# benfred/implicit

Hardware: AMD Instinct MI355X
Metric: ALS user+item updates/sec per iteration (factors=128); top-k recs/sec (higher is better)
Workload: dtype f32; 1 GPU; BASELINE configs[2]: last.fm-360K-shaped synthetic CSR, ALS CG cg_steps=3; users=358868, items=292385, nnz=17308340, factors=128, solver=cg, cg_steps=3

## Files before the change

implicit_amd/csrc/als_cg_fixup.hip:

```cpp
#include <type_traits>

#include "als_qtile.h"
#include "common.h"

namespace imp {

template <int F, typename ST>
__global__ __launch_bounds__(256) void als_cg_fault_fixup_kernel(const unsigned *__restrict__ fault_count,
                                                                 const unsigned *__restrict__ fault_rows, int capacity,
                                                                 const int32_t *__restrict__ indptr,
                                                                 const int32_t *__restrict__ indices,
                                                                 const float *__restrict__ data, ST *__restrict__ X,
                                                                 const ST *__restrict__ Y, const float *__restrict__ A0, int cg_steps,
                                                                 unsigned long long *total) {
  constexpr int FC = F / 64, WAVES = 4, U = 4;
  __shared__ float vecs[WAVES][F];
  const int n = min((int)fault_count[0], capacity);
  if (n == 0) return;
  if (blockIdx.x == 0 && threadIdx.x == 0) __hip_atomic_fetch_add(total, (unsigned long long)n, __ATOMIC_RELAXED, __HIP_MEMORY_SCOPE_SYSTEM);
  const int lane = threadIdx.x & 63, wave = threadIdx.x >> 6;
  float *vec = vecs[wave];
  auto load_vec = [&](const ST *row, float (&v)[FC]) {
#pragma unroll
    for (int c = 0; c < FC; ++c) v[c] = load1(row + FC * lane + c);
  };
  auto apply = [&](bool first, int rb, int re, const float (&v)[FC], float (&acc)[FC]) {
#pragma unroll
    for (int c = 0; c < FC; ++c) vec[FC * lane + c] = v[c];
#pragma unroll
    for (int c = 0; c < FC; ++c) acc[c] = 0.f;
    for (int j = 0; j < F; ++j) {
      const float vj = vec[j];
#pragma unroll
      for (int c = 0; c < FC; ++c) acc[c] = fmaf(A0[(size_t)j * F + FC * lane + c], vj, acc[c]);
    }
    if (first) {
#pragma unroll
      for (int c = 0; c < FC; ++c) acc[c] = -acc[c];
    }
    for (int k0 = rb; k0 < re; k0 += U) {
      float conf[U], y[U][FC];
#pragma unroll
      for (int q = 0; q < U; ++q) {
        const int k = min(k0 + q, re - 1);
        conf[q] = data[k];
        load_vec(Y + (size_t)indices[k] * F, y[q]);
      }
#pragma unroll
      for (int q = 0; q < U; ++q) {
        if (k0 + q < re) {
          const float d = wave_allsum(dot_local<FC>(y[q], v));
          const float cm1 = fabsf(conf[q]) - 1.f;
          const float w = first ? fmaxf(conf[q], 0.f) - cm1 * d : cm1 * d;
#pragma unroll
          for (int c = 0; c < FC; ++c) acc[c] = fmaf(w, y[q][c], acc[c]);
        }
      }
    }
  };
  for (int i = blockIdx.x * WAVES + wave; i < n; i += gridDim.x * WAVES) {
    const int u = (int)fault_rows[i];
    const int rb = indptr[u], re = indptr[u + 1];
    ST *xrow = X + (size_t)u * F;
    float x[FC], r[FC], p[FC], Ap[FC];
    load_vec(xrow, x);
    apply(true, rb, re, x, r);
#pragma unroll
    for (int c = 0; c < FC; ++c) p[c] = r[c];
    float rsold = wave_allsum(dot_local<FC>(r, r));
    if (rsold < 1e-20f) continue;
    for (int it = 0; it < cg_steps; ++it) {
      apply(false, rb, re, p, Ap);
      const float alpha = rsold / wave_allsum(dot_local<FC>(p, Ap));
#pragma unroll
      for (int c = 0; c < FC; ++c) {
        x[c] = fmaf(alpha, p[c], x[c]);
        r[c] = fmaf(-alpha, Ap[c], r[c]);
      }
      const float rsnew = wave_allsum(dot_local<FC>(r, r));
      if (rsnew < 1e-20f) break;
      const float beta = rsnew / rsold;
#pragma unroll
      for (int c = 0; c < FC; ++c) p[c] = fmaf(beta, p[c], r[c]);
      rsold = rsnew;
    }
#pragma unroll
    for (int c = 0; c < FC; ++c) store1(xrow + FC * lane + c, x[c]);
  }
}

unsigned long long *fixup_total() {
  auto &c = ctx();
  if (!c.fixup_total) {
    IMP_CHECK_HIP(hipHostMalloc(reinterpret_cast<void **>(&c.fixup_total), sizeof(unsigned long long), hipHostMallocMapped));
    *c.fixup_total = 0ull;
  }
  return c.fixup_total;
}

template <int F, typename T>
void launch_cg_fixup(const unsigned *count, const unsigned *rows, int capacity, const imp_csr *C, T *X, const T *Y, const float *A0,
                     int cg_steps) {
  if (capacity <= 0) return;
  IMP_PROF("als_cg_fixup");
  als_cg_fault_fixup_kernel<F, T><<<std::min((capacity + 3) / 4, ctx().num_cus * 2), 256, 0, stream()>>>(
      count, rows, capacity, C->indptr.data(), C->indices.data(), C->data.data(), X, Y, A0, cg_steps, fixup_total());
  IMP_CHECK_HIP(hipGetLastError());
}
template void launch_cg_fixup<64, float>(const unsigned *, const unsigned *, int, const imp_csr *, float *, const float *, const float *, int);
template void launch_cg_fixup<128, float>(const unsigned *, const unsigned *, int, const imp_csr *, float *, const float *, const float *, int);
template void launch_cg_fixup<64, __half>(const unsigned *, const unsigned *, int, const imp_csr *, __half *, const __half *, const float *, int);
template void launch_cg_fixup<128, __half>(const unsigned *, const unsigned *, int, const imp_csr *, __half *, const __half *, const float *, int);


}
```

implicit_amd/csrc/als_cg_nm.hip:

```cpp
#include "als_qf_common.h"
#include "common.h"
#include "wave_ops.h"

namespace imp {

namespace {

typedef _Float16 half8 __attribute__((ext_vector_type(8)));
typedef _Float16 half2v __attribute__((ext_vector_type(2)));
typedef float f32x16 __attribute__((ext_vector_type(16)));
typedef float f32x4v __attribute__((ext_vector_type(4)));
typedef unsigned u32x4 __attribute__((ext_vector_type(4)));

template <int F> struct NmShape;
template <> struct NmShape<128> {
  static constexpr int M = 32, KG = 2, NACC = 16;
  using acc_t = f32x16;
  __device__ static __forceinline__ acc_t mfma(half8 a, half8 b, acc_t c) { return __builtin_amdgcn_mfma_f32_32x32x16_f16(a, b, c, 0, 0, 0); }
  __device__ static __forceinline__ int row(int lane, int e) { return (e & 3) + 8 * (e >> 2) + 4 * (lane >> 5); }
  __device__ static __forceinline__ int col(int lane) { return lane & 31; }
};
template <> struct NmShape<64> {
  static constexpr int M = 16, KG = 4, NACC = 4;
  using acc_t = f32x4v;
// ... 22 lines not shown

__device__ __forceinline__ void split_pair(float x0, float x1, unsigned &hi, unsigned &lo) {
  const f32x2 v = {x0, x1};
  const half2v h = __builtin_convertvector(v, half2v);
  const f32x2 r = v - __builtin_convertvector(h, f32x2);
  const half2v l = __builtin_convertvector(r, half2v);
  hi = __builtin_bit_cast(unsigned, h);
  lo = __builtin_bit_cast(unsigned, l);
}
__device__ __forceinline__ unsigned pack_pair(float x0, float x1) {
  const f32x2 v = {x0, x1};
  return __builtin_bit_cast(unsigned, __builtin_convertvector(v, half2v));
}
__device__ __forceinline__ float comp(const float4 &v, int c) { return c == 0 ? v.x : c == 1 ? v.y : c == 2 ? v.z : v.w; }

template <int F> __global__ void nm_gram_image_kernel(const float *__restrict__ A0, float *__restrict__ img, int *__restrict__ ctl,
                                                      float y_rows, int forced_k, float reg = 0.f) {
  using L = NmLayout<F>;
  if (blockIdx.x == 0 && threadIdx.x < 64) {
    float d = 0.f;
    for (int j = threadIdx.x; j < F; j += 64) d = fmaxf(d, A0[(size_t)j * F + j]);
    d = wave_allmax(d);
    if (threadIdx.x == 0) {
      int k = 0;
      const float rms = sqrtf((d + reg) / fmaxf(y_rows, 1.f));
      if (rms > 0.f && rms < 8.f) k = min((int)floorf(log2f(8.f / rms)), 16);
      ctl[0] = 0;
      ctl[1] = forced_k >= 0 ? forced_k : k;
      ctl[2] = 0;
      ctl[3] = 0;
    }
  }
  for (int e = blockIdx.x * blockDim.x + threadIdx.x; e < L::IMG; e += gridDim.x * blockDim.x) {
    const int n = e % L::TS, m = (e / L::TS) % L::M, t = e / (L::TS * L::M);
    img[e] = n < L::M ? A0[(size_t)(4 * m + t / 4) * F + 4 * n + t % 4] + ((m == n && t / 4 == t % 4) ? reg : 0.f) : 0.f;
  }
}

__device__ __forceinline__ void lds_barrier() { asm volatile("s_waitcnt lgkmcnt(0)\n\ts_barrier" ::: "memory"); }

template <int F, typename T, bool TRIM = false>
__device__ __forceinline__ void nm_build(const int32_t *__restrict__ indices, const float *__restrict__ data, const T *__restrict__ Y,
                                         const float *__restrict__ gram_img, bool whole, int begin, int end, float *smem, float *bvec,
                                         int tid, int ko, int scale_k) {
  using S = NmShape<F>;
  using L = NmLayout<F>;
  constexpr bool kHalf = !std::is_same<T, float>::value;
  const int lane = tid & 63, wave = __builtin_amdgcn_readfirstlane(tid >> 6);
  const int a = lane % S::M, g = lane / S::M;
  const int first = wave < 2 ? 3 * wave : 2 * wave + 2;
  const int n_slots = wave < 2 ? 3 : 2;
  int tI[L::kSlots], tJ[L::kSlots];
#pragma unroll
  for (int k = 0; k < L::kSlots; ++k) {
    const int t = min(first + k, L::kTiles - 1);
    tI[k] = t < 1 ? 0 : t < 3 ? 1 : t < 6 ? 2 : 3;
    tJ[k] = t - tI[k] * (tI[k] + 1) / 2;
  }
// ... 196 lines not shown
      float v = b4[c];
      if constexpr (S::KG == 4) v += __shfl_xor(v, 16, 64);
      v += __shfl_xor(v, 32, 64);
      if (g == 0) bstage[wave * F + c * L::M + a] = v;
    }
    float *img = smem;
    const int n = S::col(lane);
#pragma unroll
    for (int k = 0; k < L::kSlots; ++k) {
      if (k < n_slots) {
        const int I = tI[k], J = tJ[k];
        float gv[S::NACC];
#pragma unroll
        for (int e = 0; e < S::NACC; ++e) gv[e] = 0.f;
        if (whole) {
#pragma unroll
          for (int e = 0; e < S::NACC; ++e) gv[e] = gram_img[L::at(I, J, S::row(lane, e), n)];
        }
#pragma unroll
        for (int e = 0; e < S::NACC; ++e) {
          const int m = S::row(lane, e);
          const float v = fmaf(acc[k][e], unscale2, gv[e]);
          img[L::at(I, J, m, n)] = v;
          if (I != J) img[L::at(J, I, n, m)] = v;
        }
      }
    }
  }
  __syncthreads();
}

template <int F, typename T>
// ... 221 lines not shown
    const float x2 = fmaf(-q3.z, x3, z.z) * q2.z;
    const float x1 = fmaf(-q3.y, x3, fmaf(-q2.y, x2, z.y)) * q1.y;
    const float x0 = fmaf(-q3.x, x3, fmaf(-q2.x, x2, fmaf(-q1.x, x1, z.x))) * q0.x;
    if (tid < 4 * kb) {
      const float *col = img + (size_t)(4 * kb) * LDL + tid;
      bvec[tid] = fmaf(-col[3 * LDL], x3, fmaf(-col[2 * LDL], x2, fmaf(-col[LDL], x1, fmaf(-col[0], x0, bvec[tid]))));
    }
    if (tid == 0) *reinterpret_cast<float4 *>(xs + 4 * kb) = make_float4(x0, x1, x2, x3);
    __syncthreads();
  }
  CHOL_TICK(4);
  if (tid < F) xrow[tid] = xs[tid];
  return false;
}

template <int F, typename T, bool CHOL = false>
__global__ __launch_bounds__(256, 2) void als_cg_nm_kernel(const LongPlanDev plan, const int32_t *__restrict__ indices,
                                                           const float *__restrict__ data, T *__restrict__ X, const T *__restrict__ Y,
                                                           const float *__restrict__ gram_img, int cg_steps, float *__restrict__ partial,
                                                           int *__restrict__ ticket,
                                                           unsigned *__restrict__ fix_rows,
                                                           int ko) {
  using L = NmLayout<F>;
  extern __shared__ __attribute__((aligned(16))) float smem[];
  __shared__ int next_item;
  float *img = smem, *bvec = img + L::kVec, *pv = bvec + F, *parts = pv + F, *red = parts + L::NP * F;
  const int tid = threadIdx.x;
  const int scale_k = __builtin_amdgcn_readfirstlane(ticket[1]);
  for (int s = blockIdx.x; s < plan.n_seg;) {
    const int li = plan.seg_row[s];
    const int begin = plan.seg_begin[s], end = plan.seg_end[s];
    const bool whole = plan.row_seg[li + 1] - plan.row_seg[li] == 1;
    __syncthreads();
    nm_build<F, T>(indices, data, Y, gram_img, whole, begin, end, smem, bvec, tid, ko, scale_k);
    if (tid < F) {
      const float *bstage = bvec + 2 * F + L::NP * F + 64;
      bvec[tid] = (bstage[tid] + bstage[F + tid]) + (bstage[2 * F + tid] + bstage[3 * F + tid]);
    }
    __syncthreads();
    int drawn = 0;
    if (tid == 0) drawn = (int)gridDim.x + atomicAdd(ticket, 1);
    if (!(ko & 4)) {
      if (whole) {
        bool bad = false;
        if constexpr (CHOL) bad = nm_chol<F>(img, bvec, pv, X + (size_t)plan.rows[li] * F, tid, NoGram{});
        else bad = nm_cg<F, T>(img, bvec, pv, parts, red, X + (size_t)plan.rows[li] * F, cg_steps, tid);
        if (bad && tid == 0) fix_rows[atomicAdd(ticket + 2, 1)] = (unsigned)plan.rows[li];
      } else {
        float *out = partial + (size_t)s * (L::IMG + F);
        for (int e = tid; e < L::IMG / 4; e += 256) reinterpret_cast<float4 *>(out)[e] = reinterpret_cast<const float4 *>(img)[e];
        if (tid < F) out[L::IMG + tid] = bvec[tid];
      }
    }
    if (tid == 0) next_item = drawn;
    __syncthreads();
    s = next_item;
  }
}

template <int F>
__global__ __launch_bounds__(256) void als_cg_nm_reduce_kernel(const LongPlanDev plan, int n_multi, const float *__restrict__ gram_img,
                                                               float *__restrict__ partial) {
// ... 16 lines not shown
#pragma unroll
        for (int q = 0; q < 8; ++q) sum.x += v[q].x, sum.y += v[q].y, sum.z += v[q].z, sum.w += v[q].w;
      }
      for (; s < s1; ++s) {
        const float4 v = base[(size_t)s * stride];
        sum.x += v.x, sum.y += v.y, sum.z += v.z, sum.w += v.w;
      }
      base[(size_t)s0 * stride] = sum;
    }
  }
}

template <int F, typename T, bool CHOL = false>
__global__ __launch_bounds__(256) void als_cg_nm_finish_kernel(const LongPlanDev plan, int n_multi, T *__restrict__ X, int cg_steps,
                                                               const float *__restrict__ partial, int *__restrict__ ctl,
                                                               unsigned *__restrict__ fix_rows) {
  using L = NmLayout<F>;
  extern __shared__ __attribute__((aligned(16))) float smem[];
  float *img = smem, *bvec = img + L::kVec, *pv = bvec + F, *parts = pv + F, *red = parts + L::NP * F;
  const int tid = threadIdx.x;
  for (int li = blockIdx.x; li < n_multi; li += gridDim.x) {
    const float *in = partial + (size_t)plan.row_seg[li] * (L::IMG + F);
    __syncthreads();
    for (int e = tid; e < L::IMG / 4; e += 256) reinterpret_cast<float4 *>(img)[e] = reinterpret_cast<const float4 *>(in)[e];
    if (tid < F) bvec[tid] = in[L::IMG + tid];
    __syncthreads();
    bool bad = false;
    if constexpr (CHOL) bad = nm_chol<F>(img, bvec, pv, X + (size_t)plan.rows[li] * F, tid, NoGram{});
    else bad = nm_cg<F, T>(img, bvec, pv, parts, red, X + (size_t)plan.rows[li] * F, cg_steps, tid);
    if (bad && tid == 0) fix_rows[atomicAdd(ctl + 2, 1)] = (unsigned)plan.rows[li];
  }
}

template <int F>
__global__ __launch_bounds__(256, 2) void als_chol_nm_rows_kernel(const int32_t *__restrict__ order, int first, int count,
                                                                  const int32_t *__restrict__ indptr, const int32_t *__restrict__ indices,
                                                                  const float *__restrict__ data, float *__restrict__ X,
                                                                  const float *__restrict__ Y, const float *__restrict__ gram_img,
                                                                  int *__restrict__ ctl, unsigned *__restrict__ fix_rows) {
  using L = NmLayout<F>;
  extern __shared__ __attribute__((aligned(16))) float smem[];
  __shared__ int next_item;
  float *img = smem, *bvec = img + L::kVec, *pv = bvec + F;
  const int tid = threadIdx.x;
  const int scale_k = __builtin_amdgcn_readfirstlane(ctl[1]);
// ... 19 lines not shown
    if (tid == 0) atomicAdd(&g_chol_nm_stats[5], 1ull);
#endif
    int drawn = 0;
    if (tid == 0) drawn = (int)gridDim.x + atomicAdd(ctl + 3, 1);
    const bool bad = nm_chol<F>(img, bvec, pv, X + (size_t)u * F, tid, gb);
    if (bad && tid == 0) fix_rows[atomicAdd(ctl + 2, 1)] = (unsigned)u;
    if (tid == 0) next_item = drawn;
    __syncthreads();
    i = next_item;
  }
}

template <int F, typename T> void launch_nm(const imp_csr *C, T *X, const T *Y, size_t y_rows, const float *A0, int cg_steps) {
  const LongPlan &lp = C->plan_nm;
  if (lp.n_seg <= 0) return;
  using L = NmLayout<F>;
  static_assert(L::IMG % 4 == 0, "the image is copied in 16-byte pieces");
  const size_t lds = L::lds_floats * sizeof(float);
  const int n_multi = C->nm_multi_rows, n_multi_seg = C->nm_multi_segs;
  auto &ws = ctx().long_ws;
  const size_t need = (size_t)L::IMG + (size_t)n_multi_seg * (L::IMG + F);
  if (ws.size < need) ws.alloc(need);
  float *gram_img = ws.data(), *partial = gram_img + L::IMG;
  auto &tk = ctx().nm_ticket;
  if (tk.size < 4) tk.alloc(4, true);
  auto &fix = ctx().nm_fix_rows;
  if (fix.size < (size_t)lp.n_long) fix.alloc((size_t)lp.n_long);
  LongPlanDev plan = lp.dev(C->order.data());
  auto kern = als_cg_nm_kernel<F, T>;
  auto fin = als_cg_nm_finish_kernel<F, T>;
  IMP_CHECK_HIP(hipFuncSetAttribute(reinterpret_cast<const void *>(kern), hipFuncAttributeMaxDynamicSharedMemorySize, (int)lds));
  IMP_CHECK_HIP(hipFuncSetAttribute(reinterpret_cast<const void *>(fin), hipFuncAttributeMaxDynamicSharedMemorySize, (int)lds));
  {
    IMP_PROF("als_cg_nm_rows");
    constexpr int forced_k = -1;
    nm_gram_image_kernel<F><<<(L::IMG + 255) / 256, 256, 0, stream()>>>(A0, gram_img, tk.data(), (float)y_rows, std::min(forced_k, 16));
    const int grid = std::min(lp.n_seg, ctx().num_cus * 2);
    constexpr int ko = 0;
    kern<<<grid, 256, lds, stream()>>>(plan, C->indices.data(), C->data.data(), X, Y, gram_img, cg_steps, partial, tk.data(), fix.data(), ko);
    IMP_CHECK_HIP(hipGetLastError());
  }
  if (n_multi > 0) {
    IMP_PROF("als_cg_nm_finish");
    als_cg_nm_reduce_kernel<F><<<std::min(n_multi * 16, ctx().num_cus * 16), 256, 0, stream()>>>(plan, n_multi, gram_img, partial);
    fin<<<std::min(n_multi, ctx().num_cus * 2), 256, lds, stream()>>>(plan, n_multi, X, cg_steps, partial, tk.data(), fix.data());
    IMP_CHECK_HIP(hipGetLastError());
  }
  launch_cg_fixup<F, T>(reinterpret_cast<const unsigned *>(tk.data() + 2), fix.data(), lp.n_long, C, X, Y, A0, cg_steps);
}

}

CholNmList least_squares_cholesky_nm(const imp_csr *C, float *X, const float *Y, size_t y_rows, const float *YtY, float reg) {
  constexpr int F = 128;
  using L = NmLayout<F>;
  const LongPlan &lp = C->plan_nm;
  const int32_t *b = C->bin_start;
  const size_t lds = (L::lds_floats + 128) * sizeof(float);
  const int n_multi = C->nm_multi_rows, n_multi_seg = C->nm_multi_segs;
  auto &ws = ctx().long_ws;
  const size_t need = (size_t)L::IMG + (size_t)n_multi_seg * (L::IMG + F);
  if (ws.size < need) ws.alloc(need);
  float *gram_img = ws.data(), *partial = gram_img + L::IMG;
// ... 1 lines not shown
  if (tk.size < 4) tk.alloc(4, true);
  auto &fix = ctx().nm_fix_rows;
  const int capacity = C->nonempty();
  if (fix.size < (size_t)std::max(capacity, 1)) fix.alloc((size_t)std::max(capacity, 1));
  constexpr int forced_k = -1;
  {
    IMP_PROF("als_cholesky_nm_long");
    nm_gram_image_kernel<F><<<(L::IMG + 255) / 256, 256, 0, stream()>>>(YtY, gram_img, tk.data(), (float)y_rows, std::min(forced_k, 16), reg);
    if (lp.n_seg > 0) {
      LongPlanDev plan = lp.dev(C->order.data());
      auto kern = als_cg_nm_kernel<F, float, true>;
      auto fin = als_cg_nm_finish_kernel<F, float, true>;
      IMP_CHECK_HIP(hipFuncSetAttribute(reinterpret_cast<const void *>(kern), hipFuncAttributeMaxDynamicSharedMemorySize, (int)lds));
      IMP_CHECK_HIP(hipFuncSetAttribute(reinterpret_cast<const void *>(fin), hipFuncAttributeMaxDynamicSharedMemorySize, (int)lds));
      kern<<<std::min(lp.n_seg, ctx().num_cus * 2), 256, lds, stream()>>>(plan, C->indices.data(), C->data.data(), X, Y, gram_img, -1, partial,
                                                                          tk.data(), fix.data(), 0);
      if (n_multi > 0) {
        als_cg_nm_reduce_kernel<F><<<std::min(n_multi * 16, ctx().num_cus * 16), 256, 0, stream()>>>(plan, n_multi, gram_img, partial);
        fin<<<std::min(n_multi, ctx().num_cus * 2), 256, lds, stream()>>>(plan, n_multi, X, -1, partial, tk.data(), fix.data());
      }
    }
    IMP_CHECK_HIP(hipGetLastError());
  }
  const int count = b[7] - b[1];
  if (count > 0) {
    IMP_PROF("als_cholesky_nm_rows");
    auto rk = als_chol_nm_rows_kernel<F>;
    IMP_CHECK_HIP(hipFuncSetAttribute(reinterpret_cast<const void *>(rk), hipFuncAttributeMaxDynamicSharedMemorySize, (int)lds));
    rk<<<std::min(count, ctx().num_cus * 2), 256, lds, stream()>>>(C->order.data(), b[1], count, C->indptr.data(), C->indices.data(),
                                                                    C->data.data(), X, Y, gram_img, tk.data(), fix.data());
    IMP_CHECK_HIP(hipGetLastError());
#ifdef CHOL_NM_STATS
    {
      unsigned long long h[8], z[8] = {0, 0, 0, 0, 0, 0, 0, 0};
// ... 22 lines not shown
```

implicit_amd/csrc/common.h:

```cpp
#ifndef IMPLICIT_AMD_CSRC_COMMON_H_
#define IMPLICIT_AMD_CSRC_COMMON_H_

#include <hip/hip_runtime.h>

#include <climits>
#include <cstdint>
#include <cstdio>
#include <memory>
#include <mutex>
#include <optional>
#include <stdexcept>
#include <string>
#include <vector>

#include "../../include/implicit_hip.h"
#include "csr_schedule.h"
#include "team_tickets.h"

namespace imp {

struct out_of_range_error : std::runtime_error {
  using std::runtime_error::runtime_error;
};

// ... 141 lines not shown
  void *pin_stage = nullptr;
  size_t pin_stage_bytes = 0;
  hipEvent_t pin_stage_ev = nullptr;
  DeviceArray<float> gram_ws;
  DeviceArray<float> long_ws;
  PaddedSystem pad;
  DeviceArray<double> loss_buf;
  DeviceArray<unsigned long long> chol_failed;
  DeviceArray<float> barrier_word;
  unsigned long long *fixup_total = nullptr;
  DeviceArray<float> w256_ws;
  DeviceArray<unsigned> nm_fix_rows;
  DeviceArray<unsigned> chain_counters;
  ChainTickets chain_tickets;
  DeviceArray<int> nm_ticket;
  DeviceArray<unsigned long long> bpr_stats;
  DeviceArray<float> lmf_ws;
  DeviceArray<double> knn_acc;
  DeviceArray<int32_t> knn_touched;
  int knn_cols = -1;
};
inline hipStream_t stream() { return ctx().stream; }
void note_device_write(const void *dst, size_t bytes);
struct DerivedCache {
  const void *src = nullptr;
  size_t bytes = 0;
};
void register_derived_cache(DerivedCache *c);
void unregister_derived_cache(DerivedCache *c);

// ... 71 lines not shown
  imp::DeviceArray<int32_t> row, col;
  imp::DeviceArray<float> data;
};

namespace imp {
struct PaddedViews {
  imp_matrix X, Y, YtY;
};
PaddedViews pad_in(const imp_matrix *X, const imp_matrix *Y, const imp_matrix *YtY, size_t rows_of_X, int F, bool reuse_y);
void pad_out(imp_matrix *X, size_t rows_of_X, int F);
struct CholNmList {
  const unsigned *count, *rows;
  int capacity;
};
CholNmList least_squares_cholesky_nm(const imp_csr *C, float *X, const float *Y, size_t y_rows, const float *YtY, float reg);
template <int F, typename T>
void launch_cg_fixup(const unsigned *count, const unsigned *rows, int capacity, const imp_csr *C, T *X, const T *Y, const float *A0,
                     int cg_steps);
}

#endif
```

implicit_amd/csrc/containers.hip:

```cpp
#include <hip/hip_fp16.h>

#include <algorithm>
#include <cstring>
#include <map>
#include <mutex>
#include <thread>

#include "common.h"

namespace imp {

static thread_local std::string g_last_error;
void set_last_error(const std::string &msg) { g_last_error = msg; }

static std::mutex g_ctx_mutex;
static auto &g_contexts = *new std::map<int, std::unique_ptr<Context>>;

Context &ctx() {
  int dev = 0;
  IMP_CHECK_HIP(hipGetDevice(&dev));
  std::lock_guard<std::mutex> lock(g_ctx_mutex);
  auto it = g_contexts.find(dev);
  if (it == g_contexts.end()) {
    auto c = std::make_unique<Context>();
// ... 521 lines not shown
    for (int k = 0; k < NC; ++k) {
      if (count[k] < 0 || count[k] >= ChainTickets::kMaxCount || teams_per_workgroup[k] <= 0)
        throw std::invalid_argument("host_chain_tickets: a class holds 0 .. 2^30 - 1 rows and a workgroup at least one team");
      c[k] = count[k], n[k] = teams_per_workgroup[k];
      for (int q = 0; q < NQ; ++q) t.next[k][q] = next[k * NQ + q];
    }
    t.launch(c, workgroups, n, b);
    for (int k = 0; k < NC; ++k)
      for (int q = 0; q < NQ; ++q) {
        draws[k * NQ + q] = t.next[k][q] - next[k * NQ + q];
        next[k * NQ + q] = t.next[k][q], base[k * NQ + q] = b[k][q];
      }
  });
}

int imp_matrix_create(size_t rows, size_t cols, const void *host_data, size_t itemsize, imp_matrix **out) {
  return guarded([&] {
    imp_matrix *m = new_matrix(rows, cols, itemsize, host_data == nullptr);
    std::unique_ptr<imp_matrix> guard(m);
    if (host_data && m->bytes()) {
      IMP_CHECK_HIP(hipMemcpyAsync(m->data, host_data, m->bytes(), hipMemcpyHostToDevice, stream()));
    }
    sync();
    *out = guard.release();
  });
}

int imp_matrix_wrap_device(size_t rows, size_t cols, void *device_ptr, size_t itemsize, imp_matrix **out) {
  return guarded([&] {
    if (itemsize != 4 && itemsize != 2) throw std::invalid_argument("invalid itemsize for Matrix (must be 2 or 4)");
// ... 392 lines not shown
```

implicit_amd/csrc/team_tickets.h:

```cpp
#ifndef IMPLICIT_AMD_CSRC_TEAM_TICKETS_H_
#define IMPLICIT_AMD_CSRC_TEAM_TICKETS_H_

#include <algorithm>
#include <cstdint>

namespace imp {

struct ChainTickets {
  static constexpr int kClasses = 3;
  static constexpr int kQueues = 8;
  static constexpr int kCounterStride = 64;
  static constexpr int32_t kMaxCount = 1 << 30;
  uint32_t next[kClasses][kQueues] = {};

  static int32_t queue_rows(int32_t count, int q) { return count > q ? (count - q + kQueues - 1) / kQueues : 0; }
  static int32_t queue_workgroups(int32_t workgroups, int q) { return queue_rows(workgroups, q); }
  static uint32_t draws(int32_t count, int32_t teams) {
    if (count <= 0 || teams <= 0) return 0u;
    const int64_t n = teams, c = count;
    const int64_t inside = std::max<int64_t>(0, c - 4 * n);
    const int64_t past = std::min<int64_t>(n, std::max<int64_t>(0, c - 3 * n));
    return (uint32_t)(inside + past);
  }
  void launch(const int32_t (&count)[kClasses], int32_t workgroups, const int32_t (&teams_per_workgroup)[kClasses],
              uint32_t (&base)[kClasses][kQueues]) {
    for (int c = 0; c < kClasses; ++c)
      for (int q = 0; q < kQueues; ++q) {
        base[c][q] = next[c][q];
        next[c][q] += draws(queue_rows(count[c], q), queue_workgroups(workgroups, q) * teams_per_workgroup[c]);
      }
  }
};

}

#endif
```

implicit_amd/gpu/_hip.py:

```python
import ctypes
import os

_HERE = os.path.dirname(os.path.abspath(__file__))
from .. import _libpath

LIB_PATH = _libpath.OVERRIDE or os.path.join(os.path.dirname(_HERE), "libimplicit_hip.so")

c_void_pp = ctypes.POINTER(ctypes.c_void_p)
c_i32_p = ctypes.POINTER(ctypes.c_int32)
c_f32_p = ctypes.POINTER(ctypes.c_float)

IMP_OK, IMP_INVALID_ARGUMENT, IMP_OUT_OF_RANGE, IMP_RUNTIME_ERROR = 0, 1, 2, 3

_SIGNATURES = {
    "imp_get_device_count": [ctypes.POINTER(ctypes.c_int)],
    "imp_set_device": [ctypes.c_int],
    "imp_get_device": [ctypes.POINTER(ctypes.c_int)],
    "imp_set_oversubscribe": [ctypes.c_int],
    "imp_get_oversubscribe": [ctypes.POINTER(ctypes.c_int)],
    "imp_set_deferred_sync": [ctypes.c_int],
    "imp_debug_occupy": [ctypes.c_int, ctypes.c_int],
    "imp_debug_core_clock": [ctypes.c_int, ctypes.POINTER(ctypes.c_double)],
    "imp_device_synchronize": [],
    "imp_solver_fixup_rows": [ctypes.POINTER(ctypes.c_ulonglong), ctypes.c_int],
    "imp_mem_get_info": [ctypes.POINTER(ctypes.c_size_t), ctypes.POINTER(ctypes.c_size_t)],
    "imp_release_workspaces": [],
    "imp_host_csr_transpose": [ctypes.c_int32, ctypes.c_int32, ctypes.c_int64, ctypes.c_void_p, ctypes.c_void_p, ctypes.c_void_p,
                               ctypes.c_void_p, ctypes.c_void_p, ctypes.c_void_p, ctypes.c_int],
    "imp_host_csr_plan": [ctypes.c_int32, ctypes.c_int32, ctypes.c_void_p, ctypes.c_void_p, ctypes.c_int32, ctypes.c_int32,
                          ctypes.c_int32, ctypes.c_int32, ctypes.c_int, ctypes.c_void_p, ctypes.c_void_p, ctypes.c_void_p,
                          ctypes.c_int64, ctypes.c_void_p, ctypes.c_void_p, ctypes.c_void_p, ctypes.c_void_p, ctypes.c_void_p,
                          ctypes.c_void_p],
    "imp_host_chain_tickets": [ctypes.c_void_p, ctypes.c_void_p, ctypes.c_int32, ctypes.c_void_p, ctypes.c_void_p, ctypes.c_void_p],
    "imp_matrix_create": [ctypes.c_size_t, ctypes.c_size_t, ctypes.c_void_p, ctypes.c_size_t, c_void_pp],
    "imp_matrix_wrap_device": [ctypes.c_size_t, ctypes.c_size_t, ctypes.c_void_p, ctypes.c_size_t, c_void_pp],
    "imp_matrix_row": [ctypes.c_void_p, ctypes.c_size_t, c_void_pp],
    "imp_matrix_slice": [ctypes.c_void_p, ctypes.c_size_t, ctypes.c_size_t, c_void_pp],
    "imp_matrix_gather": [ctypes.c_void_p, ctypes.c_void_p, c_void_pp],
    "imp_matrix_resize": [ctypes.c_void_p, ctypes.c_size_t, ctypes.c_size_t],
    "imp_matrix_assign_rows": [ctypes.c_void_p, ctypes.c_void_p, ctypes.c_void_p],
    "imp_matrix_astype": [ctypes.c_void_p, ctypes.c_size_t, c_void_pp],
    "imp_matrix_calculate_norms": [ctypes.c_void_p, c_void_pp],
    "imp_matrix_to_host": [ctypes.c_void_p, ctypes.c_void_p],
    "imp_matrix_from_host": [ctypes.c_void_p, ctypes.c_void_p],
    "imp_matrix_copy_rows": [ctypes.c_void_p, ctypes.c_size_t, ctypes.c_void_p, ctypes.c_size_t, ctypes.c_size_t],
    "imp_matrix_shape": [ctypes.c_void_p, ctypes.POINTER(ctypes.c_size_t), ctypes.POINTER(ctypes.c_size_t),
                         ctypes.POINTER(ctypes.c_size_t)],
    "imp_matrix_device_ptr": [ctypes.c_void_p, c_void_pp],
# ... 115 lines not shown
```

implicit_amd/utils.py:

```python
import time
import warnings

import numpy as np
import scipy.sparse


class ParameterWarning(Warning):
    """Raised (as a warning) when an input had to be converted (implicit/utils.py:155-156)."""


def check_csr(user_items):
    if isinstance(user_items, scipy.sparse.csr_matrix):
        return user_items
    kind = type(user_items).__name__
    t0 = time.time()
    converted = user_items.tocsr()
    warnings.warn(
        f"Method expects CSR input, and was passed {kind} instead. "
        f"Converting to CSR took {time.time() - t0} seconds",
        ParameterWarning,
    )
    return converted


# ... 84 lines not shown
    out.update({k: v[:out["n_seg"]] for k, v in segs.items()})
    return out


def chain_tickets(state, counts, workgroups, teams_per_workgroup=(1, 2, 4)):
    from .gpu._hip import check, lib

    assert state.dtype == np.uint32 and state.shape == (3, 8) and state.flags.c_contiguous
    counts = np.ascontiguousarray(counts, dtype=np.int32)
    teams = np.ascontiguousarray(teams_per_workgroup, dtype=np.int32)
    assert counts.shape == teams.shape == (3,)
    base, draws = np.empty((3, 8), np.uint32), np.empty((3, 8), np.uint32)
    check(lib().imp_host_chain_tickets(state.ctypes.data, counts.ctypes.data, int(workgroups), teams.ctypes.data, base.ctypes.data,
                                       draws.ctypes.data))
    return base, draws
```

include/implicit_hip.h:

```cpp
#ifndef IMPLICIT_HIP_H_
#define IMPLICIT_HIP_H_

#include <stddef.h>
#include <stdint.h>

#ifdef __cplusplus
extern "C" {
#endif

typedef enum {
  IMP_OK = 0,
  IMP_INVALID_ARGUMENT = 1,
  IMP_OUT_OF_RANGE = 2,
  IMP_RUNTIME_ERROR = 3
} imp_status;

typedef struct imp_matrix imp_matrix;
typedef struct imp_intvector imp_intvector;
typedef struct imp_csr imp_csr;
typedef struct imp_coo imp_coo;
typedef struct imp_solver imp_solver;
typedef struct imp_knn imp_knn;
typedef struct imp_random imp_random;
typedef struct imp_comm imp_comm;
// ... 11 lines not shown
int imp_solver_fixup_rows(unsigned long long *count, int reset);
int imp_mem_get_info(size_t *free_bytes, size_t *total_bytes);
int imp_release_workspaces(void);
const char *imp_version(void);

int imp_host_csr_transpose(int32_t rows, int32_t cols, int64_t nonzeros, const int32_t *indptr, const int32_t *indices,
                           const float *data, int32_t *t_indptr, int32_t *t_indices, float *t_data, int threads);

int imp_host_csr_plan(int32_t rows, int32_t cols, const int32_t *indptr, const int32_t *indices, int32_t segment, int32_t stripe,
                      int32_t nm_segment, int32_t num_cus, int which, int32_t *order, int32_t *bin_start, int32_t *row_seg,
                      int64_t seg_capacity, int32_t *seg_row, int32_t *seg_begin, int32_t *seg_end, int32_t *seg_exec,
                      int32_t *xcd_start, int32_t *info);

int imp_host_chain_tickets(uint32_t *next, const int32_t *count, int32_t workgroups, const int32_t *teams_per_workgroup, uint32_t *base,
                           uint32_t *draws);

int imp_matrix_create(size_t rows, size_t cols, const void *host_data, size_t itemsize, imp_matrix **out);
int imp_matrix_wrap_device(size_t rows, size_t cols, void *device_ptr, size_t itemsize, imp_matrix **out);
int imp_matrix_row(const imp_matrix *m, size_t rowid, imp_matrix **out);
int imp_matrix_slice(const imp_matrix *m, size_t start, size_t end, imp_matrix **out);
int imp_matrix_gather(const imp_matrix *m, const imp_intvector *rowids, imp_matrix **out);
int imp_matrix_resize(imp_matrix *m, size_t rows, size_t cols);
int imp_matrix_assign_rows(imp_matrix *m, const imp_intvector *rowids, const imp_matrix *other);
int imp_matrix_astype(const imp_matrix *m, size_t itemsize, imp_matrix **out);
int imp_matrix_calculate_norms(const imp_matrix *m, imp_matrix **out);
int imp_matrix_to_host(const imp_matrix *m, void *host_out);
int imp_matrix_from_host(imp_matrix *m, const void *host_in);
int imp_matrix_copy_rows(imp_matrix *dst, size_t dst_row, const imp_matrix *src, size_t src_row, size_t rows);
int imp_matrix_shape(const imp_matrix *m, size_t *rows, size_t *cols, size_t *itemsize);
int imp_matrix_device_ptr(const imp_matrix *m, void **ptr);
// ... 95 lines not shown
```

Baseline: 175.1 million updates/s.

## Fold NM gram-image and CG fixup kernels into the main and finish kernels

Removes the separate gram-image preparation kernel and the standalone CG fault-fixup kernel. The main NM CG kernel now computes the operand scale itself, writes the gram image only when multi-segment rows exist, and reads the row-major gram directly for whole rows. Failed rows are fixed inside the finish kernel, which now always launches. Ticket counters are made monotonic across launches with a host-tracked base and ping-pong fault lists, so no per-call counter reset is needed. This trades two kernel launches and a reset for extra work in the kernels and more bookkeeping complexity.

```diff
diff --git a/implicit_amd/csrc/als_cg_fixup.h b/implicit_amd/csrc/als_cg_fixup.h
--- /dev/null
+++ b/implicit_amd/csrc/als_cg_fixup.h
@@ -0,0 +1,80 @@
+#ifndef IMPLICIT_AMD_CSRC_ALS_CG_FIXUP_H_
+#define IMPLICIT_AMD_CSRC_ALS_CG_FIXUP_H_
+
+#include "als_qtile.h"
+#include "wave_ops.h"
+
+namespace imp {
+
+template <int F, typename ST>
+__device__ __forceinline__ void cg_fixup_row(float *vec, int rb, int re, const int32_t *__restrict__ indices, const float *__restrict__ data,
+                                             ST *xrow, const ST *__restrict__ Y, const float *__restrict__ A0, int cg_steps) {
+  constexpr int FC = F / 64, U = 4;
+  const int lane = threadIdx.x & 63;
+  auto load_vec = [&](const ST *row, float (&v)[FC]) {
+#pragma unroll
+    for (int c = 0; c < FC; ++c) v[c] = load1(row + FC * lane + c);
+  };
+  auto apply = [&](bool first, const float (&v)[FC], float (&acc)[FC]) {
+#pragma unroll
+    for (int c = 0; c < FC; ++c) vec[FC * lane + c] = v[c];
+#pragma unroll
+    for (int c = 0; c < FC; ++c) acc[c] = 0.f;
+    for (int j = 0; j < F; ++j) {
+      const float vj = vec[j];
+#pragma unroll
+      for (int c = 0; c < FC; ++c) acc[c] = fmaf(A0[(size_t)j * F + FC * lane + c], vj, acc[c]);
+    }
+    if (first) {
+#pragma unroll
+      for (int c = 0; c < FC; ++c) acc[c] = -acc[c];
+    }
+    for (int k0 = rb; k0 < re; k0 += U) {
+      float conf[U], y[U][FC];
+#pragma unroll
+      for (int q = 0; q < U; ++q) {
+        const int k = min(k0 + q, re - 1);
+        conf[q] = data[k];
+        load_vec(Y + (size_t)indices[k] * F, y[q]);
+      }
+#pragma unroll
+      for (int q = 0; q < U; ++q) {
+        if (k0 + q < re) {
+          const float d = wave_allsum(dot_local<FC>(y[q], v));
+          const float cm1 = fabsf(conf[q]) - 1.f;
+          const float w = first ? fmaxf(conf[q], 0.f) - cm1 * d : cm1 * d;
+#pragma unroll
+          for (int c = 0; c < FC; ++c) acc[c] = fmaf(w, y[q][c], acc[c]);
+        }
+      }
+    }
+  };
+  float x[FC], r[FC], p[FC], Ap[FC];
+  load_vec(xrow, x);
+  apply(true, x, r);
+#pragma unroll
+  for (int c = 0; c < FC; ++c) p[c] = r[c];
+  float rsold = wave_allsum(dot_local<FC>(r, r));
+  if (rsold < 1e-20f) return;
+  for (int it = 0; it < cg_steps; ++it) {
+    apply(false, p, Ap);
+    const float alpha = rsold / wave_allsum(dot_local<FC>(p, Ap));
+#pragma unroll
+    for (int c = 0; c < FC; ++c) {
+      x[c] = fmaf(alpha, p[c], x[c]);
+      r[c] = fmaf(-alpha, Ap[c], r[c]);
+    }
+    const float rsnew = wave_allsum(dot_local<FC>(r, r));
+    if (rsnew < 1e-20f) break;
+    const float beta = rsnew / rsold;
+#pragma unroll
+    for (int c = 0; c < FC; ++c) p[c] = fmaf(beta, p[c], r[c]);
+    rsold = rsnew;
+  }
+#pragma unroll
+  for (int c = 0; c < FC; ++c) store1(xrow + FC * lane + c, x[c]);
+}
+
+}
+
+#endif
diff --git a/implicit_amd/csrc/als_cg_fixup.hip b/implicit_amd/csrc/als_cg_fixup.hip
--- a/implicit_amd/csrc/als_cg_fixup.hip
+++ b/implicit_amd/csrc/als_cg_fixup.hip
@@ -1,93 +1,6 @@
-#include <type_traits>
-
-#include "als_qtile.h"
 #include "common.h"
 
 namespace imp {
-
-template <int F, typename ST>
-__global__ __launch_bounds__(256) void als_cg_fault_fixup_kernel(const unsigned *__restrict__ fault_count,
-                                                                 const unsigned *__restrict__ fault_rows, int capacity,
-                                                                 const int32_t *__restrict__ indptr,
-                                                                 const int32_t *__restrict__ indices,
-                                                                 const float *__restrict__ data, ST *__restrict__ X,
-                                                                 const ST *__restrict__ Y, const float *__restrict__ A0, int cg_steps,
-                                                                 unsigned long long *total) {
-  constexpr int FC = F / 64, WAVES = 4, U = 4;
-  __shared__ float vecs[WAVES][F];
-  const int n = min((int)fault_count[0], capacity);
-  if (n == 0) return;
-  if (blockIdx.x == 0 && threadIdx.x == 0) __hip_atomic_fetch_add(total, (unsigned long long)n, __ATOMIC_RELAXED, __HIP_MEMORY_SCOPE_SYSTEM);
-  const int lane = threadIdx.x & 63, wave = threadIdx.x >> 6;
-  float *vec = vecs[wave];
-  auto load_vec = [&](const ST *row, float (&v)[FC]) {
-#pragma unroll
-    for (int c = 0; c < FC; ++c) v[c] = load1(row + FC * lane + c);
-  };
-  auto apply = [&](bool first, int rb, int re, const float (&v)[FC], float (&acc)[FC]) {
-#pragma unroll
-    for (int c = 0; c < FC; ++c) vec[FC * lane + c] = v[c];
-#pragma unroll
-    for (int c = 0; c < FC; ++c) acc[c] = 0.f;
-    for (int j = 0; j < F; ++j) {
-      const float vj = vec[j];
-#pragma unroll
-      for (int c = 0; c < FC; ++c) acc[c] = fmaf(A0[(size_t)j * F + FC * lane + c], vj, acc[c]);
-    }
-    if (first) {
-#pragma unroll
-      for (int c = 0; c < FC; ++c) acc[c] = -acc[c];
-    }
-    for (int k0 = rb; k0 < re; k0 += U) {
-      float conf[U], y[U][FC];
-#pragma unroll
-      for (int q = 0; q < U; ++q) {
-        const int k = min(k0 + q, re - 1);
-        conf[q] = data[k];
-        load_vec(Y + (size_t)indices[k] * F, y[q]);
-      }
-#pragma unroll
-      for (int q = 0; q < U; ++q) {
-        if (k0 + q < re) {
-          const float d = wave_allsum(dot_local<FC>(y[q], v));
-          const float cm1 = fabsf(conf[q]) - 1.f;
-          const float w = first ? fmaxf(conf[q], 0.f) - cm1 * d : cm1 * d;
-#pragma unroll
-          for (int c = 0; c < FC; ++c) acc[c] = fmaf(w, y[q][c], acc[c]);
-        }
-      }
-    }
-  };
-  for (int i = blockIdx.x * WAVES + wave; i < n; i += gridDim.x * WAVES) {
-    const int u = (int)fault_rows[i];
-    const int rb = indptr[u], re = indptr[u + 1];
-    ST *xrow = X + (size_t)u * F;
-    float x[FC], r[FC], p[FC], Ap[FC];
-    load_vec(xrow, x);
-    apply(true, rb, re, x, r);
-#pragma unroll
-    for (int c = 0; c < FC; ++c) p[c] = r[c];
-    float rsold = wave_allsum(dot_local<FC>(r, r));
-    if (rsold < 1e-20f) continue;
-    for (int it = 0; it < cg_steps; ++it) {
-      apply(false, rb, re, p, Ap);
-      const float alpha = rsold / wave_allsum(dot_local<FC>(p, Ap));
-#pragma unroll
-      for (int c = 0; c < FC; ++c) {
-        x[c] = fmaf(alpha, p[c], x[c]);
-        r[c] = fmaf(-alpha, Ap[c], r[c]);
-      }
-      const float rsnew = wave_allsum(dot_local<FC>(r, r));
-      if (rsnew < 1e-20f) break;
-      const float beta = rsnew / rsold;
-#pragma unroll
-      for (int c = 0; c < FC; ++c) p[c] = fmaf(beta, p[c], r[c]);
-      rsold = rsnew;
-    }
-#pragma unroll
-    for (int c = 0; c < FC; ++c) store1(xrow + FC * lane + c, x[c]);
-  }
-}
 
 unsigned long long *fixup_total() {
   auto &c = ctx();
@@ -98,19 +11,4 @@
   return c.fixup_total;
 }
 
-template <int F, typename T>
-void launch_cg_fixup(const unsigned *count, const unsigned *rows, int capacity, const imp_csr *C, T *X, const T *Y, const float *A0,
-                     int cg_steps) {
-  if (capacity <= 0) return;
-  IMP_PROF("als_cg_fixup");
-  als_cg_fault_fixup_kernel<F, T><<<std::min((capacity + 3) / 4, ctx().num_cus * 2), 256, 0, stream()>>>(
-      count, rows, capacity, C->indptr.data(), C->indices.data(), C->data.data(), X, Y, A0, cg_steps, fixup_total());
-  IMP_CHECK_HIP(hipGetLastError());
 }
-template void launch_cg_fixup<64, float>(const unsigned *, const unsigned *, int, const imp_csr *, float *, const float *, const float *, int);
-template void launch_cg_fixup<128, float>(const unsigned *, const unsigned *, int, const imp_csr *, float *, const float *, const float *, int);
-template void launch_cg_fixup<64, __half>(const unsigned *, const unsigned *, int, const imp_csr *, __half *, const __half *, const float *, int);
-template void launch_cg_fixup<128, __half>(const unsigned *, const unsigned *, int, const imp_csr *, __half *, const __half *, const float *, int);
-
-
-}
diff --git a/implicit_amd/csrc/als_cg_nm.hip b/implicit_amd/csrc/als_cg_nm.hip
--- a/implicit_amd/csrc/als_cg_nm.hip
+++ b/implicit_amd/csrc/als_cg_nm.hip
@@ -1,3 +1,4 @@
+#include "als_cg_fixup.h"
 #include "als_qf_common.h"
 #include "common.h"
 #include "wave_ops.h"
@@ -60,34 +61,42 @@
 }
 __device__ __forceinline__ float comp(const float4 &v, int c) { return c == 0 ? v.x : c == 1 ? v.y : c == 2 ? v.z : v.w; }
 
+template <int F> __device__ __forceinline__ int nm_operand_scale(const float *__restrict__ A0, float y_rows, int forced_k, float reg) {
+  float d = 0.f;
+  for (int j = threadIdx.x & 63; j < F; j += 64) d = fmaxf(d, A0[(size_t)j * F + j]);
+  d = wave_allmax(d);
+  int k = 0;
+  const float rms = sqrtf((d + reg) / fmaxf(y_rows, 1.f));
+  if (rms > 0.f && rms < 8.f) k = min((int)floorf(log2f(8.f / rms)), 16);
+  return forced_k >= 0 ? forced_k : k;
+}
+
+template <int F> __device__ __forceinline__ float nm_gram_image_at(const float *__restrict__ A0, int e, float reg) {
+  using L = NmLayout<F>;
+  const int n = e % L::TS, m = (e / L::TS) % L::M, t = e / (L::TS * L::M);
+  return n < L::M ? A0[(size_t)(4 * m + t / 4) * F + 4 * n + t % 4] + ((m == n && t / 4 == t % 4) ? reg : 0.f) : 0.f;
+}
+
 template <int F> __global__ void nm_gram_image_kernel(const float *__restrict__ A0, float *__restrict__ img, int *__restrict__ ctl,
-                                                      float y_rows, int forced_k, float reg = 0.f) {
+                                                      float y_rows, int forced_k, float reg) {
   using L = NmLayout<F>;
   if (blockIdx.x == 0 && threadIdx.x < 64) {
-    float d = 0.f;
-    for (int j = threadIdx.x; j < F; j += 64) d = fmaxf(d, A0[(size_t)j * F + j]);
-    d = wave_allmax(d);
+    const int k = nm_operand_scale<F>(A0, y_rows, forced_k, reg);
     if (threadIdx.x == 0) {
-      int k = 0;
-      const float rms = sqrtf((d + reg) / fmaxf(y_rows, 1.f));
-      if (rms > 0.f && rms < 8.f) k = min((int)floorf(log2f(8.f / rms)), 16);
       ctl[0] = 0;
-      ctl[1] = forced_k >= 0 ? forced_k : k;
+      ctl[1] = k;
       ctl[2] = 0;
       ctl[3] = 0;
     }
   }
-  for (int e = blockIdx.x * blockDim.x + threadIdx.x; e < L::IMG; e += gridDim.x * blockDim.x) {
-    const int n = e % L::TS, m = (e / L::TS) % L::M, t = e / (L::TS * L::M);
-    img[e] = n < L::M ? A0[(size_t)(4 * m + t / 4) * F + 4 * n + t % 4] + ((m == n && t / 4 == t % 4) ? reg : 0.f) : 0.f;
-  }
+  for (int e = blockIdx.x * blockDim.x + threadIdx.x; e < L::IMG; e += gridDim.x * blockDim.x) img[e] = nm_gram_image_at<F>(A0, e, reg);
 }
 
 __device__ __forceinline__ void lds_barrier() { asm volatile("s_waitcnt lgkmcnt(0)\n\ts_barrier" ::: "memory"); }
 
-template <int F, typename T, bool TRIM = false>
+template <int F, typename T, bool TRIM = false, bool ROWMAJOR = false>
 __device__ __forceinline__ void nm_build(const int32_t *__restrict__ indices, const float *__restrict__ data, const T *__restrict__ Y,
-                                         const float *__restrict__ gram_img, bool whole, int begin, int end, float *smem, float *bvec,
+                                         const float *__restrict__ gram, bool whole, int begin, int end, float *smem, float *bvec,
                                          int tid, int ko, int scale_k) {
   using S = NmShape<F>;
   using L = NmLayout<F>;
@@ -314,8 +323,12 @@
 #pragma unroll
         for (int e = 0; e < S::NACC; ++e) gv[e] = 0.f;
         if (whole) {
-#pragma unroll
-          for (int e = 0; e < S::NACC; ++e) gv[e] = gram_img[L::at(I, J, S::row(lane, e), n)];
+          const unsigned lane_off = (unsigned)((4 * S::row(lane, 0) + I) * F + 4 * n + J);
+#pragma unroll
+          for (int e = 0; e < S::NACC; ++e) {
+            if constexpr (ROWMAJOR) gv[e] = (gram + 4 * S::row(0, e) * F)[lane_off];
+            else gv[e] = gram[L::at(I, J, S::row(lane, e), n)];
+          }
         }
 #pragma unroll
         for (int e = 0; e < S::NACC; ++e) {
@@ -567,38 +580,67 @@
   return false;
 }
 
+struct NmCgBuildArgs {
+  unsigned base;
+  int turn;
+  float y_rows;
+  int forced_k;
+  float *gram_img;
+};
+template <typename T> struct NmCgFinishArgs {
+  const unsigned *listed, *list;
+  unsigned *listed_next;
+  const int32_t *indices;
+  const float *data;
+  const T *Y;
+  const float *A0;
+  unsigned long long *fixed;
+};
+
 template <int F, typename T, bool CHOL = false>
 __global__ __launch_bounds__(256, 2) void als_cg_nm_kernel(const LongPlanDev plan, const int32_t *__restrict__ indices,
                                                            const float *__restrict__ data, T *__restrict__ X, const T *__restrict__ Y,
-                                                           const float *__restrict__ gram_img, int cg_steps, float *__restrict__ partial,
-                                                           int *__restrict__ ticket,
-                                                           unsigned *__restrict__ fix_rows,
+                                                           const float *__restrict__ gram, int cg_steps, float *__restrict__ partial,
+                                                           int *__restrict__ ctl, unsigned *__restrict__ fix_rows, const NmCgBuildArgs cg,
                                                            int ko) {
   using L = NmLayout<F>;
   extern __shared__ __attribute__((aligned(16))) float smem[];
   __shared__ int next_item;
   float *img = smem, *bvec = img + L::kVec, *pv = bvec + F, *parts = pv + F, *red = parts + L::NP * F;
   const int tid = threadIdx.x;
-  const int scale_k = __builtin_amdgcn_readfirstlane(ticket[1]);
+  int scale_k;
+  if constexpr (CHOL) scale_k = __builtin_amdgcn_readfirstlane(ctl[1]);
+  else scale_k = __builtin_amdgcn_readfirstlane(nm_operand_scale<F>(gram, cg.y_rows, cg.forced_k, 0.f));
+  if constexpr (!CHOL) {
+    if (cg.gram_img)
+      for (int e = blockIdx.x * 256 + tid; e < L::IMG; e += gridDim.x * 256) cg.gram_img[e] = nm_gram_image_at<F>(gram, e, 0.f);
+  }
   for (int s = blockIdx.x; s < plan.n_seg;) {
     const int li = plan.seg_row[s];
     const int begin = plan.seg_begin[s], end = plan.seg_end[s];
     const bool whole = plan.row_seg[li + 1] - plan.row_seg[li] == 1;
     __syncthreads();
-    nm_build<F, T>(indices, data, Y, gram_img, whole, begin, end, smem, bvec, tid, ko, scale_k);
+    nm_build<F, T, false, !CHOL>(indices, data, Y, gram, whole, begin, end, smem, bvec, tid, ko, scale_k);
     if (tid < F) {
       const float *bstage = bvec + 2 * F + L::NP * F + 64;
       bvec[tid] = (bstage[tid] + bstage[F + tid]) + (bstage[2 * F + tid] + bstage[3 * F + tid]);
     }
     __syncthreads();
     int drawn = 0;
-    if (tid == 0) drawn = (int)gridDim.x + atomicAdd(ticket, 1);
+    if (tid == 0) {
+      if constexpr (CHOL) drawn = (int)gridDim.x + atomicAdd(ctl, 1);
+      else drawn = (int)(gridDim.x + ((unsigned)atomicAdd(ctl, 1) - cg.base));
+    }
     if (!(ko & 4)) {
       if (whole) {
-        bool bad = false;
-        if constexpr (CHOL) bad = nm_chol<F>(img, bvec, pv, X + (size_t)plan.rows[li] * F, tid, NoGram{});
-        else bad = nm_cg<F, T>(img, bvec, pv, parts, red, X + (size_t)plan.rows[li] * F, cg_steps, tid);
-        if (bad && tid == 0) fix_rows[atomicAdd(ticket + 2, 1)] = (unsigned)plan.rows[li];
+        T *xrow = X + (size_t)plan.rows[li] * F;
+        if constexpr (CHOL) {
+          const bool bad = nm_chol<F>(img, bvec, pv, xrow, tid, NoGram{});
+          if (bad && tid == 0) fix_rows[atomicAdd(ctl + 2, 1)] = (unsigned)plan.rows[li];
+        } else {
+          const bool bad = nm_cg<F, T>(img, bvec, pv, parts, red, xrow, cg_steps, tid);
+          if (bad && tid == 0) fix_rows[atomicAdd(ctl + 1 + cg.turn, 1)] = (unsigned)li;
+        }
       } else {
         float *out = partial + (size_t)s * (L::IMG + F);
         for (int e = tid; e < L::IMG / 4; e += 256) reinterpret_cast<float4 *>(out)[e] = reinterpret_cast<const float4 *>(img)[e];
@@ -645,21 +687,37 @@
 template <int F, typename T, bool CHOL = false>
 __global__ __launch_bounds__(256) void als_cg_nm_finish_kernel(const LongPlanDev plan, int n_multi, T *__restrict__ X, int cg_steps,
                                                                const float *__restrict__ partial, int *__restrict__ ctl,
-                                                               unsigned *__restrict__ fix_rows) {
+                                                               unsigned *__restrict__ fix_rows, const NmCgFinishArgs<T> cg) {
   using L = NmLayout<F>;
   extern __shared__ __attribute__((aligned(16))) float smem[];
   float *img = smem, *bvec = img + L::kVec, *pv = bvec + F, *parts = pv + F, *red = parts + L::NP * F;
   const int tid = threadIdx.x;
+  auto resolve = [&](int li, float *vec) {
+    cg_fixup_row<F, T>(vec, plan.seg_begin[plan.row_seg[li]], plan.seg_end[plan.row_seg[li + 1] - 1], cg.indices, cg.data,
+                       X + (size_t)plan.rows[li] * F, cg.Y, cg.A0, cg_steps);
+    if ((tid & 63) == 0) __hip_atomic_fetch_add(cg.fixed, 1ull, __ATOMIC_RELAXED, __HIP_MEMORY_SCOPE_SYSTEM);
+  };
+  if constexpr (!CHOL) {
+    const int n_listed = min((int)cg.listed[0], plan.n_long);
+    if (blockIdx.x == 0 && tid == 0) cg.listed_next[0] = 0u;
+    for (int i = blockIdx.x * 4 + (tid >> 6); i < n_listed; i += gridDim.x * 4)
+      resolve((int)cg.list[i], bvec + 2 * F + L::NP * F + 64 + (tid >> 6) * F);
+  }
   for (int li = blockIdx.x; li < n_multi; li += gridDim.x) {
     const float *in = partial + (size_t)plan.row_seg[li] * (L::IMG + F);
     __syncthreads();
     for (int e = tid; e < L::IMG / 4; e += 256) reinterpret_cast<float4 *>(img)[e] = reinterpret_cast<const float4 *>(in)[e];
     if (tid < F) bvec[tid] = in[L::IMG + tid];
     __syncthreads();
-    bool bad = false;
-    if constexpr (CHOL) bad = nm_chol<F>(img, bvec, pv, X + (size_t)plan.rows[li] * F, tid, NoGram{});
-    else bad = nm_cg<F, T>(img, bvec, pv, parts, red, X + (size_t)plan.rows[li] * F, cg_steps, tid);
-    if (bad && tid == 0) fix_rows[atomicAdd(ctl + 2, 1)] = (unsigned)plan.rows[li];
+    T *xrow = X + (size_t)plan.rows[li] * F;
+    if constexpr (CHOL) {
+      const bool bad = nm_chol<F>(img, bvec, pv, xrow, tid, NoGram{});
+      if (bad && tid == 0) fix_rows[atomicAdd(ctl + 2, 1)] = (unsigned)plan.rows[li];
+    } else {
+      (void)ctl, (void)fix_rows;
+      const bool bad = nm_cg<F, T>(img, bvec, pv, parts, red, xrow, cg_steps, tid);
+      if (bad && tid < 64) resolve(li, pv);
+    }
   }
 }
 
@@ -709,39 +767,47 @@
 template <int F, typename T> void launch_nm(const imp_csr *C, T *X, const T *Y, size_t y_rows, const float *A0, int cg_steps) {
   const LongPlan &lp = C->plan_nm;
   if (lp.n_seg <= 0) return;
+  if (lp.n_seg > NmTickets::kMaxSegments) throw std::invalid_argument("least_squares_cg_nm: more than 2^30 segments of long rows");
   using L = NmLayout<F>;
   static_assert(L::IMG % 4 == 0, "the image is copied in 16-byte pieces");
   const size_t lds = L::lds_floats * sizeof(float);
   const int n_multi = C->nm_multi_rows, n_multi_seg = C->nm_multi_segs;
-  auto &ws = ctx().long_ws;
+  auto &cx = ctx();
+  auto &ws = cx.long_ws;
   const size_t need = (size_t)L::IMG + (size_t)n_multi_seg * (L::IMG + F);
   if (ws.size < need) ws.alloc(need);
   float *gram_img = ws.data(), *partial = gram_img + L::IMG;
-  auto &tk = ctx().nm_ticket;
-  if (tk.size < 4) tk.alloc(4, true);
-  auto &fix = ctx().nm_fix_rows;
+  if (!cx.nm_cg_counter.data()) cx.nm_cg_counter.alloc(3, true);
+  auto &fix = cx.nm_fix_rows;
   if (fix.size < (size_t)lp.n_long) fix.alloc((size_t)lp.n_long);
   LongPlanDev plan = lp.dev(C->order.data());
   auto kern = als_cg_nm_kernel<F, T>;
   auto fin = als_cg_nm_finish_kernel<F, T>;
   IMP_CHECK_HIP(hipFuncSetAttribute(reinterpret_cast<const void *>(kern), hipFuncAttributeMaxDynamicSharedMemorySize, (int)lds));
   IMP_CHECK_HIP(hipFuncSetAttribute(reinterpret_cast<const void *>(fin), hipFuncAttributeMaxDynamicSharedMemorySize, (int)lds));
+  constexpr int forced_k = -1;
+  unsigned *ctr = cx.nm_cg_counter.data();
+  const int turn = cx.nm_cg_turn;
+  NmCgBuildArgs cg{0u, turn, (float)y_rows, std::min(forced_k, 16), n_multi > 0 ? gram_img : nullptr};
+  const NmCgFinishArgs<T> cf{ctr + 1 + turn, fix.data(), ctr + 2 - turn, C->indices.data(), C->data.data(), Y, A0, fixup_total()};
   {
     IMP_PROF("als_cg_nm_rows");
-    constexpr int forced_k = -1;
-    nm_gram_image_kernel<F><<<(L::IMG + 255) / 256, 256, 0, stream()>>>(A0, gram_img, tk.data(), (float)y_rows, std::min(forced_k, 16));
-    const int grid = std::min(lp.n_seg, ctx().num_cus * 2);
+    const int grid = std::min(lp.n_seg, cx.num_cus * 2);
     constexpr int ko = 0;
-    kern<<<grid, 256, lds, stream()>>>(plan, C->indices.data(), C->data.data(), X, Y, gram_img, cg_steps, partial, tk.data(), fix.data(), ko);
+    NmTickets after = cx.nm_cg_tickets;
+    cg.base = after.launch(lp.n_seg);
+    kern<<<grid, 256, lds, stream()>>>(plan, C->indices.data(), C->data.data(), X, Y, A0, cg_steps, partial, reinterpret_cast<int *>(ctr), fix.data(), cg, ko);
     IMP_CHECK_HIP(hipGetLastError());
-  }
-  if (n_multi > 0) {
+    cx.nm_cg_tickets = after;
+  }
+  {
     IMP_PROF("als_cg_nm_finish");
-    als_cg_nm_reduce_kernel<F><<<std::min(n_multi * 16, ctx().num_cus * 16), 256, 0, stream()>>>(plan, n_multi, gram_img, partial);
-    fin<<<std::min(n_multi, ctx().num_cus * 2), 256, lds, stream()>>>(plan, n_multi, X, cg_steps, partial, tk.data(), fix.data());
+    if (n_multi > 0) als_cg_nm_reduce_kernel<F><<<std::min(n_multi * 16, cx.num_cus * 16), 256, 0, stream()>>>(plan, n_multi, gram_img, partial);
+    const int grid = std::min(std::max(n_multi, (lp.n_long + 3) / 4), cx.num_cus * 2);
+    fin<<<grid, 256, lds, stream()>>>(plan, n_multi, X, cg_steps, partial, nullptr, nullptr, cf);
     IMP_CHECK_HIP(hipGetLastError());
-  }
-  launch_cg_fixup<F, T>(reinterpret_cast<const unsigned *>(tk.data() + 2), fix.data(), lp.n_long, C, X, Y, A0, cg_steps);
+    cx.nm_cg_turn = 1 - turn;
+  }
 }
 
 }
@@ -773,10 +839,10 @@
       IMP_CHECK_HIP(hipFuncSetAttribute(reinterpret_cast<const void *>(kern), hipFuncAttributeMaxDynamicSharedMemorySize, (int)lds));
       IMP_CHECK_HIP(hipFuncSetAttribute(reinterpret_cast<const void *>(fin), hipFuncAttributeMaxDynamicSharedMemorySize, (int)lds));
       kern<<<std::min(lp.n_seg, ctx().num_cus * 2), 256, lds, stream()>>>(plan, C->indices.data(), C->data.data(), X, Y, gram_img, -1, partial,
-                                                                          tk.data(), fix.data(), 0);
+                                                                          tk.data(), fix.data(), NmCgBuildArgs{}, 0);
       if (n_multi > 0) {
         als_cg_nm_reduce_kernel<F><<<std::min(n_multi * 16, ctx().num_cus * 16), 256, 0, stream()>>>(plan, n_multi, gram_img, partial);
-        fin<<<std::min(n_multi, ctx().num_cus * 2), 256, lds, stream()>>>(plan, n_multi, X, -1, partial, tk.data(), fix.data());
+        fin<<<std::min(n_multi, ctx().num_cus * 2), 256, lds, stream()>>>(plan, n_multi, X, -1, partial, tk.data(), fix.data(), NmCgFinishArgs<float>{});
       }
     }
     IMP_CHECK_HIP(hipGetLastError());
diff --git a/implicit_amd/csrc/common.h b/implicit_amd/csrc/common.h
--- a/implicit_amd/csrc/common.h
+++ b/implicit_amd/csrc/common.h
@@ -179,6 +179,9 @@
   DeviceArray<unsigned> chain_counters;
   ChainTickets chain_tickets;
   DeviceArray<int> nm_ticket;
+  DeviceArray<unsigned> nm_cg_counter;
+  int nm_cg_turn = 0;
+  NmTickets nm_cg_tickets;
   DeviceArray<unsigned long long> bpr_stats;
   DeviceArray<float> lmf_ws;
   DeviceArray<double> knn_acc;
@@ -280,9 +283,6 @@
   int capacity;
 };
 CholNmList least_squares_cholesky_nm(const imp_csr *C, float *X, const float *Y, size_t y_rows, const float *YtY, float reg);
-template <int F, typename T>
-void launch_cg_fixup(const unsigned *count, const unsigned *rows, int capacity, const imp_csr *C, T *X, const T *Y, const float *A0,
-                     int cg_steps);
 }
 
 #endif
diff --git a/implicit_amd/csrc/containers.hip b/implicit_amd/csrc/containers.hip
--- a/implicit_amd/csrc/containers.hip
+++ b/implicit_amd/csrc/containers.hip
@@ -559,6 +559,16 @@
   });
 }
 
+int imp_host_nm_tickets(uint32_t *next, int32_t n_seg, uint32_t *base) {
+  return guarded_host([&] {
+    if (n_seg < 0 || n_seg > NmTickets::kMaxSegments) throw std::invalid_argument("host_nm_tickets: a plan holds 0 .. 2^30 segments");
+    NmTickets t;
+    t.next = *next;
+    *base = t.launch(n_seg);
+    *next = t.next;
+  });
+}
+
 int imp_matrix_create(size_t rows, size_t cols, const void *host_data, size_t itemsize, imp_matrix **out) {
   return guarded([&] {
     imp_matrix *m = new_matrix(rows, cols, itemsize, host_data == nullptr);
diff --git a/implicit_amd/csrc/team_tickets.h b/implicit_amd/csrc/team_tickets.h
--- a/implicit_amd/csrc/team_tickets.h
+++ b/implicit_amd/csrc/team_tickets.h
@@ -32,6 +32,16 @@
   }
 };
 
+struct NmTickets {
+  static constexpr int32_t kMaxSegments = 1 << 30;
+  uint32_t next = 0;
+  uint32_t launch(int32_t n_seg) {
+    const uint32_t base = next;
+    next += (uint32_t)std::max<int32_t>(n_seg, 0);
+    return base;
+  }
+};
+
 }
 
 #endif
diff --git a/implicit_amd/gpu/_hip.py b/implicit_amd/gpu/_hip.py
--- a/implicit_amd/gpu/_hip.py
+++ b/implicit_amd/gpu/_hip.py
@@ -32,6 +32,7 @@
                           ctypes.c_int64, ctypes.c_void_p, ctypes.c_void_p, ctypes.c_void_p, ctypes.c_void_p, ctypes.c_void_p,
                           ctypes.c_void_p],
     "imp_host_chain_tickets": [ctypes.c_void_p, ctypes.c_void_p, ctypes.c_int32, ctypes.c_void_p, ctypes.c_void_p, ctypes.c_void_p],
+    "imp_host_nm_tickets": [ctypes.c_void_p, ctypes.c_int32, ctypes.c_void_p],
     "imp_matrix_create": [ctypes.c_size_t, ctypes.c_size_t, ctypes.c_void_p, ctypes.c_size_t, c_void_pp],
     "imp_matrix_wrap_device": [ctypes.c_size_t, ctypes.c_size_t, ctypes.c_void_p, ctypes.c_size_t, c_void_pp],
     "imp_matrix_row": [ctypes.c_void_p, ctypes.c_size_t, c_void_pp],
diff --git a/implicit_amd/utils.py b/implicit_amd/utils.py
--- a/implicit_amd/utils.py
+++ b/implicit_amd/utils.py
@@ -122,3 +122,12 @@
     check(lib().imp_host_chain_tickets(state.ctypes.data, counts.ctypes.data, int(workgroups), teams.ctypes.data, base.ctypes.data,
                                        draws.ctypes.data))
     return base, draws
+
+
+def nm_tickets(state, n_seg):
+    from .gpu._hip import check, lib
+
+    assert state.dtype == np.uint32 and state.shape == (1,)
+    base = np.empty(1, np.uint32)
+    check(lib().imp_host_nm_tickets(state.ctypes.data, int(n_seg), base.ctypes.data))
+    return int(base[0])
diff --git a/include/implicit_hip.h b/include/implicit_hip.h
--- a/include/implicit_hip.h
+++ b/include/implicit_hip.h
@@ -49,6 +49,8 @@
 
 int imp_host_chain_tickets(uint32_t *next, const int32_t *count, int32_t workgroups, const int32_t *teams_per_workgroup, uint32_t *base,
                            uint32_t *draws);
+
+int imp_host_nm_tickets(uint32_t *next, int32_t n_seg, uint32_t *base);
 
 int imp_matrix_create(size_t rows, size_t cols, const void *host_data, size_t itemsize, imp_matrix **out);
 int imp_matrix_wrap_device(size_t rows, size_t cols, void *device_ptr, size_t itemsize, imp_matrix **out);
```

After: 175.5 million updates/s (median of 3 runs). No clear change (+0.2%).
